# hedgepigdaniel/video-annotator

Hardware: AMD Instinct MI355X
Metric: stabilized frames/sec at 4K NV12, 1/2/4/8 GPU; remap % HBM roofline (higher is better)
Workload: dtype u8 pixels / f32 map / f64 rotations

## Files before the change

### video-annotator_amd/csrc/vstab_testhooks.cpp

```cpp
#include <algorithm>

#include "vstab_hostlogic.hpp"
#include "vstab_pipeline.hpp"
#include "vstab_track_host.hpp"

using namespace vstab;

extern "C" {
__attribute__((visibility("default"))) int vstabx_parse_records(const uint32_t *rec, int n, uint32_t seq, int expect_n, float *xy, unsigned char *status,
                                                                 int *n_out, int *next) {
    std::vector<float> pts;
    std::vector<uint8_t> st;
    int nx = 0;
    const LkParse r = lk_parse_records(rec, 0, n, seq, (size_t)expect_n, pts, st, &nx);
    for (size_t i = 0; i < st.size(); i++) xy[2 * i] = pts[2 * i], xy[2 * i + 1] = pts[2 * i + 1], status[i] = st[i];
    *n_out = (int)st.size(), *next = nx;
    return (int)r;
}
__attribute__((visibility("default"))) int vstabx_dmabuf_cache_sim(const unsigned long long *ids, const size_t *sizes, int n, int cap, long window,
                                                                    long long fail_id, long *counts, unsigned long long *bases) {
    DmaBufCache<unsigned long long> cache;
    cache.cap = cap;
    long destroys = 0, peak = 0;
    std::vector<unsigned long long> live;
    int failures = 0;
    for (int i = 0; i < n; i++) {
        uint8_t *base = nullptr;
        const unsigned long long id = ids[i];
        const bool ok = cache.lookup(id, sizes ? sizes[i] : 4096, window,
                                     [&](unsigned long long &h, uint8_t *&b) {
                                         if ((long long)id == fail_id) return false;
                                         h = id, b = reinterpret_cast<uint8_t *>(static_cast<uintptr_t>(id * 4096));
                                         live.push_back(id);
                                         return true;
                                     },
                                     [&](unsigned long long &h) {
                                         destroys++;
                                         for (size_t k = 0; k < live.size(); k++)
                                             if (live[k] == h) {
                                                 live.erase(live.begin() + (long)k);
                                                 break;
                                             }
                                     },
                                     base);
        failures += !ok;
        bases[i] = ok ? static_cast<unsigned long long>(reinterpret_cast<uintptr_t>(base)) : ~0ull;
        peak = std::max<long>(peak, (long)cache.size());
    }
    counts[0] = cache.imports, counts[1] = cache.evictions, counts[2] = (long)cache.size(), counts[3] = destroys, counts[4] = peak;
    cache.clear([&](unsigned long long &) { destroys++; });
    counts[5] = destroys;
    return failures;
}

__attribute__((visibility("default"))) int vstabx_lk_segments(const void *const *frames, const size_t *pitches, int w, int h, const float *pts, int n,
                                                               const int *seg, int n_seg, const void *const *uv, const size_t *uv_pitches,
                                                               void *const *rings, int bad_parent, uint32_t *host_rec, uint32_t *dev_rec,
                                                               uint8_t *pyr_out, void *stream) {
    if (!frames || !pitches || !pts || !seg || !host_rec || !dev_rec || w <= 0 || h <= 0 || n <= 0 || n_seg <= 0 || n_seg > Tracker::REC_BUFS)
        return fail(VSTAB_ERR_INVALID, "vstabx_lk_segments: bad argument");
    int K = 0;
    for (int s = 0; s < n_seg; s++) {
        if (seg[s] < 1 || seg[s] > LK_SEG_MAX) return fail(VSTAB_ERR_INVALID, "vstabx_lk_segments: a launch covers 1 .. LK_SEG_MAX frame pairs");
        K += seg[s];
    }
    if (K > Tracker::REC_BUFS) return fail(VSTAB_ERR_INVALID, "vstabx_lk_segments: more frame pairs than record buffers");
    if (bad_parent != -1 && (bad_parent < 1 || bad_parent >= n_seg)) return fail(VSTAB_ERR_INVALID, "vstabx_lk_segments: bad_parent is not a chained launch");
    const bool pack = uv || uv_pitches || rings;
    if (pack && (!uv || !uv_pitches || !rings)) return fail(VSTAB_ERR_INVALID, "vstabx_lk_segments: uv, uv_pitches and rings go together");
    if (pack && lk_levels(w, h) < 2) return fail(VSTAB_ERR_INVALID, "vstabx_lk_segments: a one-level pyramid has no level 1 to pack");
    for (int i = 0; i <= K; i++) {
        if (!frames[i] || pitches[i] < (size_t)w || pitches[i] >= (1u << 24) || (uint64_t)pitches[i] * (uint64_t)h >= (1ull << 32))
            return fail(VSTAB_ERR_INVALID, "vstabx_lk_segments: bad frame");
        if (pack && (!uv[i] || !rings[i] || !pack_pyr_ok(frames[i], pitches[i], uv[i], uv_pitches[i], w, h, rings[i], rings[i], (size_t)((w + 1) / 2))))
            return fail(VSTAB_ERR_INVALID, "vstabx_lk_segments: planes not aligned for the fused copy");
    }
    hipStream_t st = static_cast<hipStream_t>(stream);
    Tracker t;
    VSTAB_TRY(t.init(w, h));
    VSTAB_TRY(t.reserve_slots(n));
    const int levels = t.levels();
    size_t pyr_bytes = 0;
    for (int l = 1; l < levels; l++) pyr_bytes += (size_t)t.level_w(l) * t.level_h(l);
    std::vector<LkPyramid> pyr(K + 1);
    int built = -1;
    auto build = [&](int i) -> vstab_status {
        const int s = i % PYR_SETS;
        const uint8_t *y = static_cast<const uint8_t *>(frames[i]);
        size_t pitch = pitches[i];
        if (pack) {
            uint8_t *ring = static_cast<uint8_t *>(rings[i]);
            VSTAB_TRY(launch_pack_pyr(y, pitch, static_cast<const uint8_t *>(uv[i]), uv_pitches[i], w, h, ring, t.level1(s), t.level1_pitch(), st));
            y = ring, pitch = (size_t)w;
        }
        VSTAB_TRY(t.build_pyramid(s, y, pitch, st, nullptr, nullptr, pack));
        pyr[i] = t.pyramid(s, y, pitch);
        if (pyr_out) {
            uint8_t *o = pyr_out + pyr_bytes * i;
            for (int l = 1; l < levels; l++) {
                const size_t lw = (size_t)t.level_w(l), lh = (size_t)t.level_h(l);
                VSTAB_HIP_TRY(hipMemcpyAsync(o, pyr[i].img[l], lw * lh, hipMemcpyDeviceToHost, st));
                o += lw * lh;
            }
        }
        built = i;
        return VSTAB_OK;
    };
    std::vector<Tracker::Launch> launches(n_seg);
    std::vector<float> start(pts, pts + 2 * (size_t)n);
    int first = 0;
    for (int s = 0; s < n_seg; s++) {
        for (int i = built + 1; i <= first + seg[s]; i++) VSTAB_TRY(build(i));
        if (s == 0) {
            VSTAB_TRY(t.track_launch(&pyr[first], seg[s], start, st, false, launches[s]));
        } else {
            Tracker::Launch parent = launches[s - 1];
            if (s == bad_parent) parent.seq[parent.n_frames - 1] ^= 0x40u;
            VSTAB_TRY(t.track_launch_chained(&pyr[first], seg[s], parent, st, launches[s]));
        }
        first += seg[s];
    }
    VSTAB_HIP_TRY(hipStreamSynchronize(st));
    int k = 0;
    for (int s = 0; s < n_seg; s++)
        for (int i = 0; i < seg[s]; i++, k++) {
            std::memcpy(host_rec + (size_t)k * n * 4, t.host_records(launches[s], i), (size_t)n * 16);
            VSTAB_HIP_TRY(hipMemcpy(dev_rec + (size_t)k * n * 4, t.dev_records(launches[s], i), (size_t)n * 16, hipMemcpyDeviceToHost));
        }
    return VSTAB_OK;
}

__attribute__((visibility("default"))) int vstabx_corners_fused(const void *gray, size_t pitch, int w, int h, double quality, unsigned int cap, unsigned int canary,
                                                                 unsigned long long *keys_out, unsigned int *counts_out, unsigned int *tile_counts,
                                                                 void *stream) {
    if (!gray || !keys_out || !counts_out || !tile_counts) return fail(VSTAB_ERR_INVALID, "vstabx_corners_fused: bad argument");
    if (w < 3 || h < 3 || pitch < (size_t)w) return fail(VSTAB_ERR_INVALID, "vstabx_corners_fused: an image is at least 3 x 3 and its pitch at least its width");
    if ((uint64_t)pitch * (uint64_t)h >= (1ull << 32) || (uint64_t)w * (uint64_t)h >= (1ull << 31))
        return fail(VSTAB_ERR_INVALID, "vstabx_corners_fused: planes of 4 GiB or more and images of 2^31 pixels or more are not supported");
    if (!(quality > 0.0) || !(quality <= 1.0)) return fail(VSTAB_ERR_INVALID, "vstabx_corners_fused: quality lies in (0, 1]");
    if (cap < 1 || cap > (1u << 24)) return fail(VSTAB_ERR_INVALID, "vstabx_corners_fused: cap is 1 .. 2^24 keys");
    if (canary < 1 || canary > (1u << 16)) return fail(VSTAB_ERR_INVALID, "vstabx_corners_fused: canary is 1 .. 2^16 keys");
    hipStream_t st = static_cast<hipStream_t>(stream);
    const size_t tiles = (size_t)div_up((unsigned)w, 64u) * div_up((unsigned)h, 31u), scratch_bytes = corners_fused_scratch_bytes(w, h);
    if (scratch_bytes != tiles * (256 * sizeof(unsigned long long) + 64 * 31 * sizeof(float) + sizeof(unsigned int)))
        return fail(VSTAB_ERR_DEVICE, "vstabx_corners_fused: the scratch layout of launch_corners_fused is not the one this hook reads");
    const size_t n_keys = (size_t)cap + canary;
    DevBuf scratch, keys, small;
    VSTAB_TRY(scratch.ensure(scratch_bytes));
    VSTAB_TRY(keys.ensure(n_keys * sizeof(unsigned long long)));
    VSTAB_TRY(small.ensure(256));
    VSTAB_HIP_TRY(hipMemsetAsync(scratch.p, 0, scratch_bytes, st));
    VSTAB_HIP_TRY(hipMemsetAsync(keys.p, 0xA5, n_keys * sizeof(unsigned long long), st));
    VSTAB_TRY(launch_corners_fused(static_cast<const uint8_t *>(gray), pitch, w, h, quality, scratch.p, keys.as<unsigned long long>(), cap, small.as<unsigned int>(), st));
    VSTAB_HIP_TRY(hipMemcpyAsync(keys_out, keys.p, n_keys * sizeof(unsigned long long), hipMemcpyDeviceToHost, st));
    VSTAB_HIP_TRY(hipMemcpyAsync(counts_out, small.as<unsigned int>() + 4, 2 * sizeof(unsigned int), hipMemcpyDeviceToHost, st));
    VSTAB_HIP_TRY(hipMemcpyAsync(tile_counts, scratch.as<uint8_t>() + (scratch_bytes - tiles * sizeof(unsigned int)), tiles * sizeof(unsigned int), hipMemcpyDeviceToHost, st));
    VSTAB_HIP_TRY(hipStreamSynchronize(st));
    return VSTAB_OK;
}

__attribute__((visibility("default"))) int vstabx_detector_counters(const vstab_handle *h, long *out) {
    if (!h || !out) return fail(VSTAB_ERR_INVALID, "vstabx_detector_counters: bad argument");
    out[0] = h->tracker.spec_over_cap(), out[1] = h->tracker.fused_overflows(), out[2] = (long)h->tracker.key_capacity();
    return VSTAB_OK;
}
}
```

### video-annotator_amd/csrc/vstab_warp_fused.hip

```cpp
#include <algorithm>
#include <climits>
#include <cmath>
#include <cstdlib>

#include "vstab_device10.hpp"
#include "vstab_warp_host.hpp"
#include "vstab_warp_tile.hpp"

namespace vstab {

#ifdef VSTAB_DEV
#define VSTAB_STAMP(k)                                                                                                   \
    if (ta.timing && lane == 0) ta.timing[((size_t)blockIdx.x * 4 + (size_t)wave) * 8 + (k)] = __builtin_amdgcn_s_memrealtime()
#else
#define VSTAB_STAMP(k)
#endif

template <int RWB, int RW, int MODE, int FMT, bool CACHED, bool SPLIT, int DEPTH = 8, int BLEND = 0>
__device__ __forceinline__ bool warp_tile(const FusedArgs &ta, uint32_t *smem, const int x0, const int y0) {
    static_assert((DEPTH == 8 && FMT < 2) || (DEPTH == 10 && FMT >= 2), "10-bit pixels leave as 16-bit BGR (FMT 2) or P010 planes (FMT 3)");
    using SrcVec = typename std::conditional<DEPTH == 10, uint4, uint2>::type;
    constexpr uint32_t BPS = DEPTH == 10 ? 2 : 1;
    constexpr int TH = 4 * RW;
    constexpr int STAGE_MAX = StageTrips<RWB, RW>::value;
    constexpr int QB = CACHED ? 0 : QMAGIC_BITS;
    constexpr bool PIX8 = DEPTH == 10 && BLEND == VSTAB_BLEND_FP16;
    constexpr int PD = PIX8 ? 2 : 1;
    constexpr bool RS = map_mode_is_rs(MODE);
    constexpr int BASE = map_mode_base(MODE);
    uint32_t *const tile = smem + 8;
    const WarpArgs &a = ta.w;
    const int tid = threadIdx.x, lane = tid & 63, wave = __builtin_amdgcn_readfirstlane(tid >> 6);
    const float rfx = rcp_refined(a.p.ofx), rfy = rcp_refined(a.p.ofy);

    VSTAB_STAMP(0);
    if (wave == 0) {
        __builtin_amdgcn_s_setprio(3);
        probe_tile<TH, STAGE_MAX, MODE, CACHED>(ta, x0, y0, lane, rfx, rfy, smem);
        __builtin_amdgcn_s_setprio(VSTAB_WARP_PRIO);
    }
    __syncthreads();
    const int bx0 = __builtin_amdgcn_readfirstlane((int)smem[0]), by0 = __builtin_amdgcn_readfirstlane((int)smem[1]);
    const int wb = __builtin_amdgcn_readfirstlane((int)smem[2]), hb = __builtin_amdgcn_readfirstlane((int)smem[3]);
    const int box_state = __builtin_amdgcn_readfirstlane((int)smem[4]);
    if constexpr (SPLIT) {
        if (box_state == 2) return false;
    }
    const bool use_lds = box_state == 1;
    const int x = x0 + lane;
    VSTAB_STAMP(1);

    const int ux_n = wb >> 3, units = use_lds ? ux_n * (hb >> 1) : 0;
#ifdef VSTAB_DEV
    const int pw = (wb + ta.lds_pad) * PD;
#else
    const int pw = wb * PD;
#endif
    SrcVec y0w[STAGE_MAX], y1w[STAGE_MAX], uvw[STAGE_MAX];
    int ldsoff[STAGE_MAX];
    constexpr int ZERO_BLOCK = 1 << 24;
    if (use_lds) {
        const float rn = __builtin_amdgcn_rcpf((float)ux_n);
        int uy = (int)((float)tid * rn), ux = tid - uy * ux_n;
        if (ux < 0) ux += ux_n, uy--;
        if (ux >= ux_n) ux -= ux_n, uy++;
        int sy_ = (int)(256.0f * rn), sx_ = 256 - sy_ * ux_n;
        if (sx_ < 0) sx_ += ux_n, sy_--;
        if (sx_ >= ux_n) sx_ -= ux_n, sy_++;
        const uint32_t pitch_y = (uint32_t)a.pitch_y, pitch_uv = (uint32_t)a.pitch_uv;
#pragma unroll
        for (int it = 0; it < STAGE_MAX; it++) {
            if (it > 0 && units <= it * 256) {
                y0w[it] = y1w[it] = uvw[it] = SrcVec(), ldsoff[it] = -1;
                continue;
            }
            const bool valid = tid + it * 256 < units;
            const int gx = bx0 + 8 * ux, gy = by0 + 2 * uy;
            const bool inside = (uint32_t)gx < (uint32_t)(a.sw & ~7) && (uint32_t)gy < (uint32_t)a.sh;
            const uint32_t cx = (uint32_t)min(max(gx, 0), (a.sw & ~7) - 8), cy = (uint32_t)min(max(gy, 0), a.sh - 2);
            const uint32_t oy = __umul24(cy, pitch_y) + cx * BPS, ouv = __umul24(cy >> 1, pitch_uv) + cx * BPS;
            y0w[it] = *reinterpret_cast<const SrcVec *>(a.y + oy);
            y1w[it] = *reinterpret_cast<const SrcVec *>(a.y + (oy + pitch_y));
            uvw[it] = *reinterpret_cast<const SrcVec *>(a.uv + ouv);
            ldsoff[it] = valid ? (__mul24(2 * uy, pw) + 8 * PD * ux) | (inside ? 0 : ZERO_BLOCK) : -1;
            ux += sx_, uy += sy_;
            if (ux >= ux_n) ux -= ux_n, uy++;
        }
    } else {
#pragma unroll
        for (int it = 0; it < STAGE_MAX; it++) y0w[it] = y1w[it] = uvw[it] = SrcVec(), ldsoff[it] = -1;
    }

    VSTAB_STAMP(2);
    int qxb[RW], qyb[RW];
    {
        int unused_cx[RW / 2], unused_cy[RW / 2];
        const float unused_qm[4] = {QMAGIC, QMAGIC, QMAGIC, QMAGIC};
        map_phase<RW, MODE, CACHED, false>(ta, x, y0, wave, lane, rfx, rfy, qxb, qyb, unused_cx, unused_cy, unused_qm);
    }
#pragma unroll
    for (int j = 0; j < RW; j++) asm volatile("" : "+v"(qxb[j]), "+v"(qyb[j]) : : "memory");

    VSTAB_STAMP(3);
    if (use_lds) {
#pragma unroll
        for (int it = 0; it < STAGE_MAX; it++) {
            if (ldsoff[it] >= ZERO_BLOCK) {
                uint32_t *d = tile + (ldsoff[it] - ZERO_BLOCK);
                const uint4 z = make_uint4(0, 0, 0, 0);
#pragma unroll
                for (int q = 0; q < 2 * PD; q++) *reinterpret_cast<uint4 *>(d + 4 * q) = z, *reinterpret_cast<uint4 *>(d + pw + 4 * q) = z;
#ifdef VSTAB_DEV
            } else if (DEPTH == 8 && ldsoff[it] >= 0 && (ta.ablate & 4)) {
                uint32_t *d = tile + ldsoff[it];
                *reinterpret_cast<uint4 *>(d) = make_uint4(y0w[it].x, y0w[it].y, uvw[it].x, uvw[it].y);
                *reinterpret_cast<uint4 *>(d + 4) = make_uint4(y0w[it].y, y0w[it].x, uvw[it].x, uvw[it].y);
                *reinterpret_cast<uint4 *>(d + pw) = make_uint4(y1w[it].x, y1w[it].y, uvw[it].x, uvw[it].y);
                *reinterpret_cast<uint4 *>(d + pw + 4) = make_uint4(y1w[it].y, y1w[it].x, uvw[it].y, uvw[it].x);
#endif
            } else if (ldsoff[it] >= 0) {
                uint32_t *d = tile + ldsoff[it];
                if constexpr (DEPTH == 10) {
                    const uint32_t ya[4] = {y0w[it].x, y0w[it].y, y0w[it].z, y0w[it].w}, yb[4] = {y1w[it].x, y1w[it].y, y1w[it].z, y1w[it].w};
                    const uint32_t cw[4] = {uvw[it].x, uvw[it].y, uvw[it].z, uvw[it].w};
#pragma unroll
                    for (int half = 0; half < 2; half++) {
                        const ChromaTerm c0 = chroma_term10(cw[2 * half]), c1 = chroma_term10(cw[2 * half + 1]);
                        if constexpr (PIX8) {
                            const uint32_t la = ya[2 * half], lb = ya[2 * half + 1], ma = yb[2 * half], mb = yb[2 * half + 1];
                            const uint2 a0 = pack_bgr10h((int)((la & 0xffffu) >> 6), c0), a1 = pack_bgr10h((int)(la >> 22), c0);
                            const uint2 a2 = pack_bgr10h((int)((lb & 0xffffu) >> 6), c1), a3 = pack_bgr10h((int)(lb >> 22), c1);
                            const uint2 b0 = pack_bgr10h((int)((ma & 0xffffu) >> 6), c0), b1 = pack_bgr10h((int)(ma >> 22), c0);
                            const uint2 b2 = pack_bgr10h((int)((mb & 0xffffu) >> 6), c1), b3 = pack_bgr10h((int)(mb >> 22), c1);
                            *reinterpret_cast<uint4 *>(d + 8 * half) = make_uint4(a0.x, a0.y, a1.x, a1.y);
                            *reinterpret_cast<uint4 *>(d + 8 * half + 4) = make_uint4(a2.x, a2.y, a3.x, a3.y);
                            *reinterpret_cast<uint4 *>(d + pw + 8 * half) = make_uint4(b0.x, b0.y, b1.x, b1.y);
                            *reinterpret_cast<uint4 *>(d + pw + 8 * half + 4) = make_uint4(b2.x, b2.y, b3.x, b3.y);
                            continue;
                        }
                        uint4 r0, r1;
                        r0.x = pack_bgr10((int)((ya[2 * half] & 0xffffu) >> 6), c0), r0.y = pack_bgr10((int)(ya[2 * half] >> 22), c0);
                        r0.z = pack_bgr10((int)((ya[2 * half + 1] & 0xffffu) >> 6), c1), r0.w = pack_bgr10((int)(ya[2 * half + 1] >> 22), c1);
                        r1.x = pack_bgr10((int)((yb[2 * half] & 0xffffu) >> 6), c0), r1.y = pack_bgr10((int)(yb[2 * half] >> 22), c0);
                        r1.z = pack_bgr10((int)((yb[2 * half + 1] & 0xffffu) >> 6), c1), r1.w = pack_bgr10((int)(yb[2 * half + 1] >> 22), c1);
                        *reinterpret_cast<uint4 *>(d + 4 * half) = r0;
                        *reinterpret_cast<uint4 *>(d + pw + 4 * half) = r1;
                    }
                } else
#pragma unroll
                for (int half = 0; half < 2; half++) {
                    const uint32_t cw = half ? uvw[it].y : uvw[it].x, ya = half ? y0w[it].y : y0w[it].x, yb = half ? y1w[it].y : y1w[it].x;
                    const ChromaTerm c0 = chroma_term_folded(cw & 255, (cw >> 8) & 255);
                    const ChromaTerm c1 = chroma_term_folded((cw >> 16) & 255, cw >> 24);
                    uint4 r0, r1;
                    r0.x = pack_bgrx(ya & 255, c0), r0.y = pack_bgrx((ya >> 8) & 255, c0);
                    r0.z = pack_bgrx((ya >> 16) & 255, c1), r0.w = pack_bgrx(ya >> 24, c1);
                    r1.x = pack_bgrx(yb & 255, c0), r1.y = pack_bgrx((yb >> 8) & 255, c0);
                    r1.z = pack_bgrx((yb >> 16) & 255, c1), r1.w = pack_bgrx(yb >> 24, c1);
                    *reinterpret_cast<uint4 *>(d + 4 * half) = r0;
                    *reinterpret_cast<uint4 *>(d + pw + 4 * half) = r1;
                }
            }
        }
    }
    VSTAB_STAMP(4);
    __syncthreads();
    VSTAB_STAMP(5);

    const bool col_live = x < a.dw;
    uint32_t out[RW];
    {
        int cx = bx0 + (QB >> 5), cy = by0 + (QB >> 5);
        asm("" : "+s"(cx), "+s"(cy));
        const uint32_t wlim = use_lds ? (uint32_t)(wb - 1) : 0u, hlim = (uint32_t)(hb - 1);
        int Xr[RW], Yr[RW];
        const uint32_t wb4 = (uint32_t)pw << 2;
        uint32_t tile_lds = (uint32_t)(uintptr_t)(__attribute__((address_space(3))) uint32_t *)tile;
        asm("" : "+s"(tile_lds));
        uint32_t mxx = 0, mxy = 0;
#pragma unroll
        for (int j = 0; j < RW; j++) {
            Xr[j] = (qxb[j] >> 5) - cx, Yr[j] = (qyb[j] >> 5) - cy;
            mxx = max(mxx, (uint32_t)Xr[j]), mxy = max(mxy, (uint32_t)Yr[j]);
        }
        if (!__builtin_amdgcn_ballot_w64(mxx >= wlim || mxy >= hlim)) {
            constexpr int TG = RW < TAP_GROUP ? RW : TAP_GROUP;
            if constexpr (PIX8) {
#pragma unroll
                for (int j0 = 0; j0 < RW; j0 += TG) {
                    uint2 t0[TG], t1[TG], t2[TG], t3[TG];
#pragma unroll
                    for (int j = 0; j < TG; j++) {
                        uint32_t ax8, au;
                        asm("v_lshl_add_u32 %0, %1, 3, %2" : "=v"(ax8) : "v"(Xr[j0 + j]), "s"(tile_lds));
                        asm("v_mad_u32_u24 %0, %1, %2, %3" : "=v"(au) : "v"(Yr[j0 + j]), "s"(wb4), "v"(ax8));
                        const LdsPair *u = reinterpret_cast<const LdsPair *>(au), *l = reinterpret_cast<const LdsPair *>(au + wb4);
                        const u32x2 v0 = u[0], v1 = u[1], v2 = l[0], v3 = l[1];
                        t0[j] = make_uint2(v0.x, v0.y), t1[j] = make_uint2(v1.x, v1.y), t2[j] = make_uint2(v2.x, v2.y), t3[j] = make_uint2(v3.x, v3.y);
                    }
#pragma unroll
                    for (int j = 0; j < TG; j++) out[j0 + j] = blend_bgr10h(t0[j], t1[j], t2[j], t3[j], qxb[j0 + j] & 31, qyb[j0 + j] & 31);
                }
            } else
#pragma unroll
            for (int j0 = 0; j0 < RW; j0 += TG) {
                uint32_t t0[TG], t1[TG], t2[TG], t3[TG];
#pragma unroll
                for (int j = 0; j < TG; j++) {
                    uint32_t ax4, au;
                    asm("v_lshl_add_u32 %0, %1, 2, %2" : "=v"(ax4) : "v"(Xr[j0 + j]), "s"(tile_lds));
                    asm("v_mad_u32_u24 %0, %1, %2, %3" : "=v"(au) : "v"(Yr[j0 + j]), "s"(wb4), "v"(ax4));
                    const LdsWord *u = reinterpret_cast<const LdsWord *>(au), *l = reinterpret_cast<const LdsWord *>(au + wb4);
                    t0[j] = u[0], t1[j] = u[1], t2[j] = l[0], t3[j] = l[1];
                }
#pragma unroll
                for (int j = 0; j < TG; j++) {
#ifdef VSTAB_DEV
                    if (ta.ablate & 2) out[j0 + j] = t0[j] ^ t1[j] ^ t2[j] ^ t3[j] ^ (qxb[j0 + j] & 31) ^ (qyb[j0 + j] & 31);
                    else
#endif
                    out[j0 + j] = DEPTH == 10 ? blend_bgr10<BLEND>(t0[j], t1[j], t2[j], t3[j], qxb[j0 + j] & 31, qyb[j0 + j] & 31)
                                              : blend_bgrx(t0[j], t1[j], t2[j], t3[j], qxb[j0 + j] & 31, qyb[j0 + j] & 31);
                }
            }
        } else {
            uint32_t slow = 0;
#pragma unroll
            for (int j = 0; j < RW; j++) {
                const bool inbox = (uint32_t)Xr[j] < wlim && (uint32_t)Yr[j] < hlim;
                uint32_t v = 0;
                if (inbox) {
                    const uint32_t *t = tile + (__mul24(Yr[j], pw) + PD * Xr[j]);
                    if constexpr (PIX8)
                        v = blend_bgr10h(make_uint2(t[0], t[1]), make_uint2(t[2], t[3]), make_uint2(t[pw], t[pw + 1]), make_uint2(t[pw + 2], t[pw + 3]), qxb[j] & 31,
                                         qyb[j] & 31);
                    else
                        v = DEPTH == 10 ? blend_bgr10<BLEND>(t[0], t[1], t[pw], t[pw + 1], qxb[j] & 31, qyb[j] & 31)
                                        : blend_bgrx(t[0], t[1], t[pw], t[pw + 1], qxb[j] & 31, qyb[j] & 31);
                }
                out[j] = v;
                const bool live = col_live && y0 + wave * RW + j < a.dh;
                slow |= (!inbox && live ? 1u : 0u) << j;
            }
            if (__builtin_amdgcn_ballot_w64(slow != 0)) {
#pragma unroll 1
                for (int j = 0; j < RW; j++) {
                    int sx = qxb[0], sy = qyb[0];
#pragma unroll
                    for (int k = 1; k < RW; k++) sx = j == k ? qxb[k] : sx, sy = j == k ? qyb[k] : sy;
                    if ((slow >> j) & 1u) {
                        const uint32_t v = DEPTH == 10 ? gather_pixel10<BLEND>(a, sx - QB, sy - QB) : gather_pixel_far(a, sx - QB, sy - QB);
#pragma unroll
                        for (int k = 0; k < RW; k++) out[k] = j == k ? v : out[k];
                    }
// ... 134 lines not shown
    return true;
}

template <int RWB, int MODE, int FMT, bool CACHED, int DEPTH = 8, int BLEND = 0>
__global__ void __launch_bounds__(256, DEPTH == 10 ? 5 : (RWB == 8 || map_mode_is_rs(MODE)) ? VSTAB_WARP_WAVES - 1 : VSTAB_WARP_WAVES) k_warp_fused(FusedArgs ta) {
    extern __shared__ __attribute__((aligned(16))) uint32_t smem[];
    constexpr int TH = 4 * RWB, TS = TH / 2;
    if (VSTAB_WARP_PRIO) __builtin_amdgcn_s_setprio(VSTAB_WARP_PRIO);
    const int k = (int)(blockIdx.x & 7u);
    const int y_lo = ta.band_y[k], y_sp = ta.split_y[k], y_hi = ta.band_y[k + 1];
    const int n_tall = ((y_sp - y_lo) / TH) * ta.tiles_x;
    const int idx = (int)(blockIdx.x >> 3);
    int x0, ys, n_half;
    if (idx < n_tall) {
        const int row = idx / ta.tiles_x;
        x0 = (idx - row * ta.tiles_x) * 64, ys = y_lo + row * TH;
        n_half = warp_tile<RWB, RWB, MODE, FMT, CACHED, true, DEPTH, BLEND>(ta, smem, x0, ys) ? 0 : 2;
    } else {
        const int i2 = idx - n_tall, row = i2 / ta.tiles_x;
        x0 = (i2 - row * ta.tiles_x) * 64, ys = y_sp + row * TS, n_half = 1;
        if (ys >= y_hi) return;
    }
#pragma unroll 1
    for (int i = 0; i < n_half; i++) warp_tile<RWB, RWB / 2, MODE, FMT, CACHED, false, DEPTH, BLEND>(ta, smem, x0, ys + i * TS);
}

}

using namespace vstab;

namespace vstab {
#ifdef VSTAB_DEV
static unsigned long long *g_dev_timing = nullptr;
extern "C" __attribute__((visibility("default"))) void vstab_dev_set_timing(void *p) { g_dev_timing = static_cast<unsigned long long *>(p); }
#endif

vstab_status launch_warp_fused10(const WarpArgs &a, const float params[17], int map_mode, int blend, const float *rot_bottom, bool p010_out, bool src_vec_ok,
                                 bool dst_vec_ok, hipStream_t st) {
    FusedArgs ta;
    fill_fused_args(ta, a, params, src_vec_ok, dst_vec_ok, nullptr, 0, rot_bottom);
    const int lds_kb = 40;
    const bool half = blend == VSTAB_BLEND_FP16;
    const int rwb = 8;
    const long tiles = (long)div_up(a.dw, 64) * div_up(a.dh, 4 * rwb);
    const dim3 grid(tile_schedule(ta, rwb, lds_kb, tiles > 1024 ? 0.5 : 0.0));
    if (half) ta.lds_capacity_px /= 2;
    const size_t lds_bytes = (size_t)lds_kb * 1024;
    vstab_status status = VSTAB_OK;
    with_map_mode(map_mode, rot_bottom != nullptr, [&](auto mode) {
        with_either<VSTAB_BLEND_FP16, VSTAB_BLEND_EXACT>(half, [&](auto blend_c) {
            with_either<3, 2>(p010_out, [&](auto fmt) {
                constexpr int MODE = decltype(mode)::value;
                if constexpr (map_mode_fish_to_pinhole(map_mode_base(MODE)))
                    launch_kernel(k_warp_fused<8, MODE, decltype(fmt)::value, false, 10, decltype(blend_c)::value>, grid, dim3(256), lds_bytes, st, ta);
                else
                    status = fail(VSTAB_ERR_INVALID, "launch_warp_fused10: the 10-bit tiled kernels serve map modes 0, 1 and 5 only");
            });
        });
    });
    if (status != VSTAB_OK) return status;
    VSTAB_HIP_TRY(hipGetLastError());
    return VSTAB_OK;
}

vstab_status launch_warp_fused(const WarpArgs &a, const float params[17], int map_mode, bool nv12_out, bool src_vec_ok, bool dst_vec_ok,
                               const void *qmap, int qpitch, const float *rot_bottom, hipStream_t st, const float *dist) {
    FusedArgs ta;
    fill_fused_args(ta, a, params, src_vec_ok, dst_vec_ok, qmap, qpitch, rot_bottom, dist);
#ifdef VSTAB_DEV
    ta.timing = g_dev_timing;
    static const int ablate = getenv("VSTAB_ABLATE") ? atoi(getenv("VSTAB_ABLATE")) : 0;
    ta.ablate = ablate;
    ta.lds_pad = getenv("VSTAB_LDS_PAD") ? atoi(getenv("VSTAB_LDS_PAD")) & ~3 : 0;
#endif
    const long tiles32 = (long)div_up(a.dw, 64) * div_up(a.dh, 32);
    int rwb = tiles32 < 1536 ? 4 : 8, lds_kb = rwb == 4 ? 20 : 40;
    double tail_rounds = (double)div_up(a.dw, 64) * div_up(a.dh, 4 * rwb) > 256.0 * (160 / lds_kb) ? 0.5 : 0.0;
#ifdef VSTAB_DEV
    if (const char *e = getenv("VSTAB_ROWS")) rwb = atoi(e) == 4 ? 4 : 8;
    if (const char *e = getenv("VSTAB_LDS_KB")) lds_kb = atoi(e);
    if (const char *e = getenv("VSTAB_TAIL_ROUNDS")) tail_rounds = atof(e);
#endif
    const size_t lds_bytes = (size_t)lds_kb * 1024;
    const dim3 grid(tile_schedule(ta, rwb, lds_kb, tail_rounds));
    if (dist) {
        if (nv12_out || qmap || rot_bottom) return fail(VSTAB_ERR_INVALID, "launch_warp_fused: the distorted-lens kernels emit BGR8 from one rotation per frame");
        with_dist_mode(map_mode, [&](auto mode) {
            with_either<8, 4>(rwb == 8, [&](auto rows) {
                launch_kernel(k_warp_fused<decltype(rows)::value, decltype(mode)::value, 0, false>, grid, dim3(256), lds_bytes, st, ta);
            });
        });
        VSTAB_HIP_TRY(hipGetLastError());
        return VSTAB_OK;
    }
    with_map_mode(qmap ? (int)VSTAB_MAP_CREATEMAP_CL : map_mode, !qmap && rot_bottom != nullptr, [&](auto mode) {
        with_bool(qmap != nullptr, [&](auto cached) {
            with_either<8, 4>(rwb == 8, [&](auto rows) {
                with_either<1, 0>(nv12_out, [&](auto fmt) {
                    constexpr int MODE = decltype(mode)::value;
                    constexpr bool CACHED = decltype(cached)::value;
                    if constexpr (!CACHED || MODE == MAP_CREATEMAP_CL)
                        launch_kernel(k_warp_fused<decltype(rows)::value, MODE, decltype(fmt)::value, CACHED>, grid, dim3(256), lds_bytes, st, ta);
                });
            });
        });
    });
    VSTAB_HIP_TRY(hipGetLastError());
    return VSTAB_OK;
}


vstab_status preload_fused_kernels() {
    hipFuncAttributes at;
    VSTAB_HIP_TRY(hipFuncGetAttributes(&at, reinterpret_cast<const void *>((&k_warp_fused<8, MAP_CREATEMAP_CL_OPENCL, 0, false, 8, 0>))));
    return VSTAB_OK;
}

}
```

### video-annotator_amd/csrc/vstab_warp_tile.hpp

```cpp
#pragma once
#include <algorithm>
#include <climits>
#include <cmath>
#include <cstdlib>

#include "vstab_device.hpp"
#include "vstab_internal.hpp"
#include "vstab_warp_args.hpp"

namespace vstab {

#ifndef VSTAB_WARP_WAVES
#define VSTAB_WARP_WAVES 7
#endif
#ifndef VSTAB_WARP_PRIO
#define VSTAB_WARP_PRIO 1
#endif
#ifndef VSTAB_MAP_GROUP
#define VSTAB_MAP_GROUP 2
#endif
#ifndef VSTAB_TAP_GROUP
#define VSTAB_TAP_GROUP 4
#endif
constexpr int MAP_GROUP = VSTAB_MAP_GROUP;
constexpr int TAP_GROUP = VSTAB_TAP_GROUP;
constexpr float QMAGIC = 12582912.0f;
constexpr int QMAGIC_BITS = 0x4B400000;

typedef short short2v __attribute__((ext_vector_type(2)));
typedef __attribute__((address_space(3))) uint32_t LdsWord;
typedef uint32_t u32x2 __attribute__((ext_vector_type(2)));
typedef __attribute__((address_space(3))) u32x2 LdsPair;

__device__ __forceinline__ uint32_t pk_min_i16(uint32_t a, uint32_t b) {
    return __builtin_bit_cast(uint32_t, __builtin_elementwise_min(__builtin_bit_cast(short2v, a), __builtin_bit_cast(short2v, b)));
}
__device__ __forceinline__ uint32_t pk_max_i16(uint32_t a, uint32_t b) {
    return __builtin_bit_cast(uint32_t, __builtin_elementwise_max(__builtin_bit_cast(short2v, a), __builtin_bit_cast(short2v, b)));
}

template <bool MAX>
__device__ __forceinline__ uint32_t wave_reduce_pk_i16(uint32_t v) {
    constexpr uint32_t ident = MAX ? 0x80008000u : 0x7fff7fffu;
#define VSTAB_STEP(ctrl, rmask)                                                                              \
    {                                                                                                        \
        const uint32_t t = (uint32_t)__builtin_amdgcn_update_dpp((int)ident, (int)v, ctrl, rmask, 0xf, false); \
        v = MAX ? pk_max_i16(v, t) : pk_min_i16(v, t);                                                       \
    }
    VSTAB_STEP(0x111, 0xf) VSTAB_STEP(0x112, 0xf) VSTAB_STEP(0x114, 0xf) VSTAB_STEP(0x118, 0xf)
    VSTAB_STEP(0x142, 0xa) VSTAB_STEP(0x143, 0xc)
#undef VSTAB_STEP
    return (uint32_t)__builtin_amdgcn_readlane((int)v, 63);
}

__device__ __forceinline__ uint32_t gather_pixel_far(const WarpArgs &a, int sx, int sy) {
    const int X = sx >> 5, Y = sy >> 5;
    if (!(X < a.sw && X + 1 >= 0 && Y < a.sh && Y + 1 >= 0)) return 0;
    return gather_pixel(a, sx, sy);
}

template <int RWB, int RW>
struct StageTrips {
    static constexpr int value = RW == 8 ? 3 : RW == 4 ? 2 : (RWB == 8 ? 2 : 1);
};

template <int TH, int STAGE_MAX, int MODE, bool CACHED, bool PLANAR = false, int BLOCK_W = 8>
__device__ __forceinline__ void probe_tile(const FusedArgs &ta, int x0, int y0, int lane, float rfx, float rfy, uint32_t *hdr) {
    constexpr bool RS = map_mode_is_rs(MODE);
    constexpr int BASE = map_mode_base(MODE);
    const WarpArgs &a = ta.w;
    int px, py;
    const int l16 = lane & 15, side = (l16 * (TH - 1) + 7) / 15;
    if (lane < 16) px = 4 * l16, py = 0;
    else if (lane < 32) px = 4 * l16 + 3, py = TH - 1;
    else if (lane < 48) px = 0, py = side;
    else px = 63, py = side;
    px = min(px, a.dw - 1 - x0), py = min(py, a.dh - 1 - y0);
    int qx, qy;
    if constexpr (CACHED) {
        const int2 q = ta.qmap[(size_t)(y0 + py) * ta.qpitch + (x0 + px)];
        qx = q.x, qy = q.y;
    } else {
        float ax, ay;
        if constexpr (BASE == MAP_CREATEMAP_CL || BASE == MAP_FISH_TO_RECT || BASE == MAP_CREATEMAP_CL_OPENCL || BASE == MAP_FISHD_TO_RECT) {
            const float vx = ((float)(x0 + px) - a.p.ocx) * rfx, vy = ((float)(y0 + py) - a.p.ocy) * rfy;
            float m[9];
#pragma unroll
            for (int k = 0; k < 9; k++) m[k] = a.p.r[k];
            if constexpr (RS) {
                const float t = (float)(y0 + py) * __builtin_amdgcn_rcpf(ta.rs_den);
#pragma unroll
                for (int k = 0; k < 9; k++) m[k] = __builtin_fmaf(t, ta.rs_d[k], a.p.r[k]);
            }
            const float wx = __builtin_fmaf(m[0], vx, __builtin_fmaf(m[1], vy, m[2]));
            const float wy = __builtin_fmaf(m[3], vx, __builtin_fmaf(m[4], vy, m[5]));
            const float wz = __builtin_fmaf(m[6], vx, __builtin_fmaf(m[7], vy, m[8]));
            const float rz = __builtin_amdgcn_rcpf(wz), ux = wx * rz, uy = wy * rz;
            const float q = __builtin_fmaf(ux, ux, uy * uy), rs = __builtin_amdgcn_rsqf(q), rad = q * rs;
            const bool inv = rad > 1.0f;
            const float t = inv ? rs : rad, s2 = t * t;
            float g = 0.0028423243202269077f;
            g = __builtin_fmaf(g, s2, -0.016053270548582077f);
            g = __builtin_fmaf(g, s2, 0.04269874095916748f);
            g = __builtin_fmaf(g, s2, -0.07508683204650879f);
            g = __builtin_fmaf(g, s2, 0.1064559817314148f);
            g = __builtin_fmaf(g, s2, -0.14205896854400635f);
            g = __builtin_fmaf(g, s2, 0.19993145763874054f);
            g = __builtin_fmaf(g, s2, -0.33333125710487366f);
            float at = __builtin_fmaf(t * s2, g, t);
            at = inv ? 1.57079637050628662109375f - at : at;
            if constexpr (BASE == MAP_FISHD_TO_RECT) {
                const Distortion &dk = ta.p32.d;
                const float a2 = at * at;
                const float pd = __builtin_fmaf(__builtin_fmaf(__builtin_fmaf(dk.k4, a2, dk.k3), a2, dk.k2), a2, dk.k1);
                at = at * __builtin_fmaf(pd, a2, 1.0f);
            }
            const float k = at * rs;
            ax = __builtin_fmaf(ux * k, ta.p32.ifx32, ta.p32.icx32), ay = __builtin_fmaf(uy * k, ta.p32.ify32, ta.p32.icy32);
            if ((BASE == MAP_FISH_TO_RECT || BASE == MAP_FISHD_TO_RECT) && !(wz > 0.0f)) ax = ay = __builtin_nanf("");
        } else {
            const float vx = div_with_rcp((float)(x0 + px) - a.p.ocx, a.p.ofx, rfx);
            const float vy = div_with_rcp((float)(y0 + py) - a.p.ocy, a.p.ofy, rfy);
            const ColTerm ct = {a.p.r[0] * vx, a.p.r[3] * vx, a.p.r[6] * vx};
            const RowTerm rt = {a.p.r[1] * vy, a.p.r[4] * vy, a.p.r[7] * vy};
            map_pixel_ex<BASE>(ta.p32, a.p, ct, rt, vx, vy, ax, ay);
        }
        qx = __float_as_int(ax + QMAGIC) - QMAGIC_BITS, qy = __float_as_int(ay + QMAGIC) - QMAGIC_BITS;
    }
    int Xc, Yc;
    asm("v_med3_i32 %0, %1, -1, %2" : "=v"(Xc) : "v"(qx >> 5), "s"(a.sw));
    asm("v_med3_i32 %0, %1, -1, %2" : "=v"(Yc) : "v"(qy >> 5), "s"(a.sh));
    const uint32_t pk = ((uint32_t)Xc & 0xffffu) | ((uint32_t)Yc << 16);
    const uint32_t mn = wave_reduce_pk_i16<false>(pk), mx = wave_reduce_pk_i16<true>(pk);
    const int mnx = (int)(short)(mn & 0xffffu), mny = (int)mn >> 16, mxx = (int)(short)(mx & 0xffffu), mxy = (int)mx >> 16;
    constexpr int LO_M = PLANAR ? 2 : 1, HI_M = PLANAR ? 5 : 2, CAP = PLANAR ? 1 : 0, BM = BLOCK_W - 1;
    const int lox = max(mnx - LO_M, -LO_M), hix = min(mxx + HI_M, a.sw + CAP), loy = max(mny - LO_M, -LO_M), hiy = min(mxy + HI_M, a.sh + CAP);
    const int bx0 = lox & ~BM, by0 = loy & ~1;
    const int wb = (hix + 1 - bx0 + BM) & ~BM, hb = (hiy + 1 - by0 + 1) & ~1;
    const bool have = mnx < a.sw && mxx >= -1 && mny < a.sh && mxy >= -1;
    const bool stageable = have && a.sw >= BLOCK_W && ta.src_vec_ok && ((a.sw & BM) == 0 || bx0 + wb <= (a.sw & ~BM));
#ifdef VSTAB_DEV
    const bool fits = (wb + ta.lds_pad) * hb <= ta.lds_capacity_px && (wb >> 3) * (hb >> 1) <= STAGE_MAX * 256;
#else
    const bool fits = wb * hb <= ta.lds_capacity_px && (wb / BLOCK_W) * (hb >> 1) <= STAGE_MAX * 256 && (!PLANAR || wb / BLOCK_W <= 64);
#endif
    if (lane == 0) {
        *reinterpret_cast<uint4 *>(hdr) = make_uint4((uint32_t)bx0, (uint32_t)by0, (uint32_t)wb, (uint32_t)hb);
        hdr[4] = stageable ? (fits ? 1u : 2u) : 0u;
    }
}

#define VSTAB_EACH _Pragma("unroll") for (int c = 0; c < NP; c++)
template <int NP, bool FISH_TO_RECT, bool DIST = false>
__device__ __forceinline__ void map_pairs_ieee(float icx32, float icy32, float ifx32, float ify32, const f32x2 (&wx)[NP], const f32x2 (&wy)[NP],
                                               const f32x2 (&wz)[NP], f32x2 (&ax)[NP], f32x2 (&ay)[NP], const Distortion &dk = Distortion()) {
    f32x2 rz[NP], e[NP], px[NP], py[NP], ex[NP], ey[NP], q[NP], y[NP], g[NP], h[NP], d[NP], rad[NP], rr[NP], t[NP], s[NP], at[NP], k[NP];
    i32x2 inv[NP];
    const f32x2 one = splat2(1.0f), half = splat2(0.5f);
    VSTAB_EACH rz[c] = (f32x2){__builtin_amdgcn_rcpf(wz[c].x), __builtin_amdgcn_rcpf(wz[c].y)};
    VSTAB_EACH e[c] = fma2(-wz[c], rz[c], one);
    VSTAB_EACH rz[c] = fma2(e[c], rz[c], rz[c]);
    VSTAB_EACH px[c] = wx[c] * rz[c], py[c] = wy[c] * rz[c];
    VSTAB_EACH ex[c] = fma2(-wz[c], px[c], wx[c]), ey[c] = fma2(-wz[c], py[c], wy[c]);
    VSTAB_EACH px[c] = fma2(ex[c], rz[c], px[c]), py[c] = fma2(ey[c], rz[c], py[c]);
    VSTAB_EACH ex[c] = fma2(-wz[c], px[c], wx[c]), ey[c] = fma2(-wz[c], py[c], wy[c]);
    VSTAB_EACH px[c] = fma2(ex[c], rz[c], px[c]), py[c] = fma2(ey[c], rz[c], py[c]);
    VSTAB_EACH q[c] = px[c] * px[c] + py[c] * py[c];
    VSTAB_EACH y[c] = (f32x2){__builtin_amdgcn_rsqf(q[c].x), __builtin_amdgcn_rsqf(q[c].y)};
    VSTAB_EACH g[c] = q[c] * y[c], h[c] = half * y[c];
    VSTAB_EACH e[c] = fma2(-h[c], g[c], half);
    VSTAB_EACH h[c] = fma2(h[c], e[c], h[c]), g[c] = fma2(g[c], e[c], g[c]);
    VSTAB_EACH d[c] = fma2(-g[c], g[c], q[c]);
    VSTAB_EACH rad[c] = fma2(d[c], h[c], g[c]);
    VSTAB_EACH rr[c] = (f32x2){__builtin_amdgcn_rcpf(rad[c].x), __builtin_amdgcn_rcpf(rad[c].y)};
    VSTAB_EACH e[c] = fma2(-rad[c], rr[c], one);
    VSTAB_EACH rr[c] = fma2(e[c], rr[c], rr[c]);
    VSTAB_EACH inv[c] = rad[c] > one, t[c] = one * rr[c];
    VSTAB_EACH e[c] = fma2(-rad[c], t[c], one);
    VSTAB_EACH t[c] = fma2(e[c], rr[c], t[c]);
    VSTAB_EACH e[c] = fma2(-rad[c], t[c], one);
    VSTAB_EACH t[c] = fma2(e[c], rr[c], t[c]);
    VSTAB_EACH t[c] = inv[c] ? t[c] : rad[c];
    VSTAB_EACH s[c] = t[c] * t[c];
    VSTAB_EACH g[c] = fma2(splat2(0.0028423243202269077f), s[c], splat2(-0.016053270548582077f));
    VSTAB_EACH g[c] = fma2(g[c], s[c], splat2(0.04269874095916748f));
    VSTAB_EACH g[c] = fma2(g[c], s[c], splat2(-0.07508683204650879f));
    VSTAB_EACH g[c] = fma2(g[c], s[c], splat2(0.1064559817314148f));
    VSTAB_EACH g[c] = fma2(g[c], s[c], splat2(-0.14205896854400635f));
    VSTAB_EACH g[c] = fma2(g[c], s[c], splat2(0.19993145763874054f));
    VSTAB_EACH g[c] = fma2(g[c], s[c], splat2(-0.33333125710487366f));
    VSTAB_EACH at[c] = fma2(t[c] * s[c], g[c], t[c]);
    VSTAB_EACH at[c] = inv[c] ? (splat2(1.57079637050628662109375f) - at[c]) + splat2(-4.37113900018624283e-8f) : at[c];
    if constexpr (DIST) {
        VSTAB_EACH s[c] = at[c] * at[c];
        VSTAB_EACH g[c] = splat2(dk.k4) * s[c];
        VSTAB_EACH g[c] = g[c] + splat2(dk.k3);
        VSTAB_EACH g[c] = g[c] * s[c];
        VSTAB_EACH g[c] = g[c] + splat2(dk.k2);
        VSTAB_EACH g[c] = g[c] * s[c];
        VSTAB_EACH g[c] = g[c] + splat2(dk.k1);
        VSTAB_EACH g[c] = g[c] * s[c];
        VSTAB_EACH g[c] = one + g[c];
        VSTAB_EACH at[c] = at[c] * g[c];
    }
    VSTAB_EACH k[c] = at[c] * rr[c];
    VSTAB_EACH e[c] = fma2(-rad[c], k[c], at[c]);
    VSTAB_EACH k[c] = fma2(e[c], rr[c], k[c]);
    VSTAB_EACH e[c] = fma2(-rad[c], k[c], at[c]);
    VSTAB_EACH k[c] = fma2(e[c], rr[c], k[c]);
    if constexpr (FISH_TO_RECT) {
        VSTAB_EACH k[c] = (q[c] == splat2(0.0f)) ? one : k[c];
    }
    VSTAB_EACH ax[c] = splat2(icx32) + (px[c] * k[c]) * splat2(ifx32), ay[c] = splat2(icy32) + (py[c] * k[c]) * splat2(ify32);
    if constexpr (FISH_TO_RECT) {
        VSTAB_EACH {
            const i32x2 ok = wz[c] > splat2(0.0f);
            ax[c] = ok ? ax[c] : splat2(__builtin_nanf("")), ay[c] = ok ? ay[c] : splat2(__builtin_nanf(""));
        }
    }
}

__device__ __forceinline__ bool map_q_irregular(uint32_t qmin, uint32_t qmax) { return qmin < 0x17800000u  || qmax > 0x67800000u ; }
template <int NP>
__device__ __forceinline__ void map_pairs_ocl(float icx32, float icy32, float ifx32, float ify32, const f32x2 (&wx)[NP], const f32x2 (&wy)[NP],
                                              const f32x2 (&wz)[NP], f32x2 (&ax)[NP], f32x2 (&ay)[NP], uint32_t &qmin, uint32_t &qmax) {
    f32x2 rz[NP], px[NP], py[NP], q[NP], rad[NP], rr[NP], t[NP], s[NP], p[NP], r[NP], k[NP];
    i32x2 inv[NP];
    VSTAB_EACH rz[c] = (f32x2){__builtin_amdgcn_rcpf(wz[c].x), __builtin_amdgcn_rcpf(wz[c].y)};
    VSTAB_EACH px[c] = wx[c] * rz[c], py[c] = wy[c] * rz[c];
    VSTAB_EACH q[c] = fma2(py[c], py[c], px[c] * px[c]);
    VSTAB_EACH rad[c] = (f32x2){__builtin_amdgcn_sqrtf(q[c].x), __builtin_amdgcn_sqrtf(q[c].y)};
// ... 189 lines not shown
```

Measured before the change: 28220.

## Add cost-weighted band scheduling and dead-tile skip for fisheye warp

Adds a host-side cost model that estimates, per tile row, how much source footprint the projection touches. It uses that estimate to place the eight band boundaries so each band gets balanced work instead of equal rows, and caches the schedule for rotations within a small angle. On the device, the probe wave now checks whether a whole tile maps well outside the source image. If so, the tile skips map and sample work and writes zeros. This trades a host-side geometric estimate and a conservative device-side guard for less imbalance and less wasted gather work, but risks wrong zero tiles if the margin heuristics are too loose.

Measured after the change: 30480 (median of 6 runs). +8.0%, better.

```diff
diff --git a/video-annotator_amd/csrc/vstab_testhooks.cpp b/video-annotator_amd/csrc/vstab_testhooks.cpp
--- a/video-annotator_amd/csrc/vstab_testhooks.cpp
+++ b/video-annotator_amd/csrc/vstab_testhooks.cpp
@@ -3,6 +3,7 @@
 #include "vstab_hostlogic.hpp"
 #include "vstab_pipeline.hpp"
 #include "vstab_track_host.hpp"
+#include "vstab_warp_bands.hpp"
 
 using namespace vstab;
 
@@ -159,6 +160,44 @@
     return VSTAB_OK;
 }
 
+__attribute__((visibility("default"))) int vstabx_weighted_bands(int dw, int dh, int rwb, int lds_kb, double tail_rounds, const uint32_t *cost, int n_cost,
+                                                                  int *out) {
+    if (!out || dw < 1 || dh < 1 || (rwb != 4 && rwb != 8) || lds_kb < 1 || !(tail_rounds >= 0.0) || n_cost < 0)
+        return fail(VSTAB_ERR_INVALID, "vstabx_weighted_bands: bad argument");
+    FusedArgs ta = {};
+    ta.w.dw = dw, ta.w.dh = dh;
+    const unsigned grid = cost ? weighted_bands(ta, rwb, lds_kb, tail_rounds, cost, n_cost) : tile_schedule(ta, rwb, lds_kb, tail_rounds);
+    for (int k = 0; k < 9; k++) out[k] = ta.band_y[k];
+    for (int k = 0; k < 8; k++) out[9 + k] = ta.split_y[k];
+    out[17] = ta.tiles_x, out[18] = (int)grid;
+    return VSTAB_OK;
+}
+__attribute__((visibility("default"))) int vstabx_band_costs(const float *params, int nan_behind, int sw, int sh, int dw, int dh, int ts, uint32_t *cost, int n_cost) {
+    if (!params || !cost || sw < 1 || sh < 1 || dw < 1 || dh < 1 || (ts != 8 && ts != 16) || n_cost != (int)div_up((unsigned)dh, (unsigned)ts))
+        return fail(VSTAB_ERR_INVALID, "vstabx_band_costs: bad argument");
+    std::vector<uint32_t> c;
+    band_costs(params, nan_behind != 0, sw, sh, dw, dh, ts, c);
+    std::copy(c.begin(), c.end(), cost);
+    return VSTAB_OK;
+}
+__attribute__((visibility("default"))) int vstabx_band_cache_run(const float *params, int n, int sw, int sh, int dw, int dh, int map_mode, int rwb, int lds_kb,
+                                                                  double tail_rounds, int *out, long *counts) {
+    if (!params || !out || !counts || n < 1 || sw < 1 || sh < 1 || dw < 1 || dh < 1 || (rwb != 4 && rwb != 8) || lds_kb < 1 || !(tail_rounds >= 0.0))
+        return fail(VSTAB_ERR_INVALID, "vstabx_band_cache_run: bad argument");
+    BandCache cache;
+    for (int i = 0; i < n; i++) {
+        FusedArgs ta = {};
+        ta.w.sw = sw, ta.w.sh = sh, ta.w.dw = dw, ta.w.dh = dh;
+        const unsigned grid = cache.schedule(ta, params + 17 * (size_t)i, map_mode, rwb, lds_kb, tail_rounds);
+        int *o = out + 19 * (size_t)i;
+        for (int k = 0; k < 9; k++) o[k] = ta.band_y[k];
+        for (int k = 0; k < 8; k++) o[9 + k] = ta.split_y[k];
+        o[17] = ta.tiles_x, o[18] = (int)grid;
+    }
+    counts[0] = cache.hits, counts[1] = cache.misses, counts[2] = (long)cache.entries.size();
+    return VSTAB_OK;
+}
+
 __attribute__((visibility("default"))) int vstabx_detector_counters(const vstab_handle *h, long *out) {
     if (!h || !out) return fail(VSTAB_ERR_INVALID, "vstabx_detector_counters: bad argument");
     out[0] = h->tracker.spec_over_cap(), out[1] = h->tracker.fused_overflows(), out[2] = (long)h->tracker.key_capacity();
diff --git a/video-annotator_amd/csrc/vstab_warp_bands.hpp b/video-annotator_amd/csrc/vstab_warp_bands.hpp
--- /dev/null
+++ b/video-annotator_amd/csrc/vstab_warp_bands.hpp
@@ -0,0 +1,139 @@
+#pragma once
+#include <array>
+#include <cmath>
+#include <cstdint>
+#include <cstring>
+#include <mutex>
+#include <vector>
+
+#include "vstab_warp_tile.hpp"
+
+namespace vstab {
+
+static inline unsigned weighted_bands(FusedArgs &ta, int rwb, int lds_kb, double tail_rounds, const uint32_t *cost, int n_cost) {
+    const unsigned even_grid = tile_schedule(ta, rwb, lds_kb, tail_rounds);
+    const WarpArgs &a = ta.w;
+    const int th = 4 * rwb, ts = th / 2;
+    const int half_rows = (int)div_up(a.dh, ts);
+    if (!cost || n_cost != half_rows) return even_grid;
+    uint64_t total = 0;
+    for (int i = 0; i < half_rows; i++) total += cost[i];
+    if (total == 0) return even_grid;
+    const int slots = 32 * std::max(1, std::min(8, (int)(160 / lds_kb)));
+    int h = 0;
+    uint64_t prefix = 0;
+    ta.band_y[0] = 0;
+    for (int k = 1; k < 8; k++) {
+        while (h < half_rows && 8 * (prefix + cost[h]) <= (uint64_t)k * total) prefix += cost[h++];
+        ta.band_y[k] = std::min(a.dh, h * ts);
+    }
+    ta.band_y[8] = a.dh;
+    int share = 0;
+    for (int k = 0; k < 8; k++) {
+        const int rows = ta.band_y[k + 1] - ta.band_y[k];
+        const int tall_rows_max = rows / th;
+        const int tail_tall_rows = (int)std::min<long>(tall_rows_max, std::lround(tail_rounds * slots / ta.tiles_x));
+        const int tall_rows = tall_rows_max - tail_tall_rows;
+        ta.split_y[k] = ta.band_y[k] + tall_rows * th;
+        const int n = tall_rows * ta.tiles_x + (int)div_up(ta.band_y[k + 1] - ta.split_y[k], ts) * ta.tiles_x;
+        share = std::max(share, n);
+    }
+    return 8u * (unsigned)share;
+}
+
+constexpr uint32_t BAND_COST_DEAD = 135, BAND_COST_LIVE = 220;
+constexpr double BAND_COST_PER_BLOCK = 0.58;
+
+static inline void band_costs(const float params[17], bool nan_behind, int sw, int sh, int dw, int dh, int ts, std::vector<uint32_t> &cost) {
+    const int tiles_x = (int)div_up(dw, 64), half_rows = (int)div_up(dh, ts);
+    const double icx = params[0], icy = params[1], ifx = params[2], ify = params[3], ocx = params[4], ocy = params[5], ofx = params[6], ofy = params[7];
+    const float *r = params + 8;
+    std::vector<double> X((size_t)(tiles_x + 1) * 2), Y((size_t)(tiles_x + 1) * 2);
+    auto corners = [&](int row, double *xo, double *yo) {
+        const double vy = ((double)std::min(row * ts, dh - 1) - ocy) / ofy;
+        for (int c = 0; c <= tiles_x; c++) {
+            const double vx = ((double)std::min(c * 64, dw - 1) - ocx) / ofx;
+            const double wx = r[0] * vx + r[1] * vy + r[2], wy = r[3] * vx + r[4] * vy + r[5], wz = r[6] * vx + r[7] * vy + r[8];
+            if (!(wz > 0.0) && (nan_behind || wz == 0.0)) {
+                xo[c] = yo[c] = NAN;
+                continue;
+            }
+            const double ux = wx / wz, uy = wy / wz, rad = std::sqrt(ux * ux + uy * uy), k = rad > 0.0 ? std::atan(rad) / rad : 1.0;
+            xo[c] = icx + ifx * ux * k, yo[c] = icy + ify * uy * k;
+        }
+    };
+    cost.assign((size_t)half_rows, 0u);
+    double *x0 = X.data(), *x1 = x0 + tiles_x + 1, *y0 = Y.data(), *y1 = y0 + tiles_x + 1;
+    corners(0, x0, y0);
+    for (int row = 0; row < half_rows; row++) {
+        corners(row + 1, x1, y1);
+        uint32_t sum = 0;
+        for (int c = 0; c < tiles_x; c++) {
+            const double xs[4] = {x0[c], x0[c + 1], x1[c], x1[c + 1]}, ys[4] = {y0[c], y0[c + 1], y1[c], y1[c + 1]};
+            double mnx = xs[0], mxx = xs[0], mny = ys[0], mxy = ys[0];
+            bool finite = true;
+            for (int i = 0; i < 4; i++) {
+                finite = finite && std::isfinite(xs[i]) && std::isfinite(ys[i]);
+                mnx = std::min(mnx, xs[i]), mxx = std::max(mxx, xs[i]), mny = std::min(mny, ys[i]), mxy = std::max(mxy, ys[i]);
+            }
+            double blocks = 64.0 * ts * 4.0 / 16.0;
+            if (finite) {
+                if (mxx < -1.0 || mnx >= (double)sw || mxy < -1.0 || mny >= (double)sh) {
+                    sum += BAND_COST_DEAD;
+                    continue;
+                }
+                const double bw = std::min(mxx + 2.0, (double)sw) - std::max(mnx - 1.0, -1.0) + 8.0;
+                const double bh = std::min(mxy + 2.0, (double)sh) - std::max(mny - 1.0, -1.0) + 2.0;
+                blocks = std::max(bw, 8.0) * std::max(bh, 2.0) / 16.0;
+            }
+            sum += BAND_COST_LIVE + (uint32_t)std::min(blocks * BAND_COST_PER_BLOCK, 4096.0);
+        }
+        cost[(size_t)row] = sum;
+        std::swap(x0, x1), std::swap(y0, y1);
+    }
+}
+
+constexpr double BAND_CACHE_ANGLE = 1.5 * 3.14159265358979323846 / 180.0;
+constexpr int BAND_CACHE_ENTRIES = 32;
+struct BandCache {
+    struct Entry {
+        float fixed[8];
+        int dims[8];
+        float rot[9];
+        int band_y[9], split_y[8];
+        unsigned grid;
+    };
+    std::mutex mu;
+    std::vector<Entry> entries;
+    size_t next = 0;
+    long hits = 0, misses = 0;
+
+    unsigned schedule(FusedArgs &ta, const float params[17], int map_mode, int rwb, int lds_kb, double tail_rounds) {
+        const WarpArgs &a = ta.w;
+        const int dims[8] = {a.sw, a.sh, a.dw, a.dh, map_mode, rwb, lds_kb, (int)std::lround(tail_rounds * 64.0)};
+        const double min_trace = 1.0 + 2.0 * std::cos(BAND_CACHE_ANGLE);
+        std::lock_guard<std::mutex> lock(mu);
+        for (const Entry &e : entries) {
+            if (std::memcmp(e.fixed, params, sizeof e.fixed) || std::memcmp(e.dims, dims, sizeof dims)) continue;
+            double tr = 0.0;
+            for (int i = 0; i < 9; i++) tr += (double)e.rot[i] * params[8 + i];
+            if (!(tr >= min_trace)) continue;
+            tile_schedule(ta, rwb, lds_kb, tail_rounds);
+            std::memcpy(ta.band_y, e.band_y, sizeof e.band_y), std::memcpy(ta.split_y, e.split_y, sizeof e.split_y);
+            hits++;
+            return e.grid;
+        }
+        misses++;
+        std::vector<uint32_t> cost;
+        band_costs(params, map_mode == MAP_FISH_TO_RECT, a.sw, a.sh, a.dw, a.dh, 2 * rwb, cost);
+        Entry e;
+        std::memcpy(e.fixed, params, sizeof e.fixed), std::memcpy(e.dims, dims, sizeof dims), std::memcpy(e.rot, params + 8, sizeof e.rot);
+        e.grid = weighted_bands(ta, rwb, lds_kb, tail_rounds, cost.data(), (int)cost.size());
+        std::memcpy(e.band_y, ta.band_y, sizeof e.band_y), std::memcpy(e.split_y, ta.split_y, sizeof e.split_y);
+        if ((int)entries.size() < BAND_CACHE_ENTRIES) entries.push_back(e);
+        else entries[next++ % BAND_CACHE_ENTRIES] = e;
+        return e.grid;
+    }
+};
+
+}
diff --git a/video-annotator_amd/csrc/vstab_warp_fused.hip b/video-annotator_amd/csrc/vstab_warp_fused.hip
--- a/video-annotator_amd/csrc/vstab_warp_fused.hip
+++ b/video-annotator_amd/csrc/vstab_warp_fused.hip
@@ -4,6 +4,7 @@
 #include <cstdlib>
 
 #include "vstab_device10.hpp"
+#include "vstab_warp_bands.hpp"
 #include "vstab_warp_host.hpp"
 #include "vstab_warp_tile.hpp"
 
@@ -28,6 +29,7 @@
     constexpr int PD = PIX8 ? 2 : 1;
     constexpr bool RS = map_mode_is_rs(MODE);
     constexpr int BASE = map_mode_base(MODE);
+    constexpr bool DEAD = !CACHED && !RS && (BASE == MAP_CREATEMAP_CL || BASE == MAP_CREATEMAP_CL_OPENCL || BASE == MAP_FISH_TO_RECT);
     uint32_t *const tile = smem + 8;
     const WarpArgs &a = ta.w;
     const int tid = threadIdx.x, lane = tid & 63, wave = __builtin_amdgcn_readfirstlane(tid >> 6);
@@ -36,7 +38,7 @@
     VSTAB_STAMP(0);
     if (wave == 0) {
         __builtin_amdgcn_s_setprio(3);
-        probe_tile<TH, STAGE_MAX, MODE, CACHED>(ta, x0, y0, lane, rfx, rfy, smem);
+        probe_tile<TH, STAGE_MAX, MODE, CACHED, false, 8, DEAD>(ta, x0, y0, lane, rfx, rfy, smem);
         __builtin_amdgcn_s_setprio(VSTAB_WARP_PRIO);
     }
     __syncthreads();
@@ -47,6 +49,7 @@
         if (box_state == 2) return false;
     }
     const bool use_lds = box_state == 1;
+    const bool dead = DEAD && box_state == 3;
     const int x = x0 + lane;
     VSTAB_STAMP(1);
 
@@ -93,7 +96,10 @@
 
     VSTAB_STAMP(2);
     int qxb[RW], qyb[RW];
-    {
+    if (dead) {
+#pragma unroll
+        for (int j = 0; j < RW; j++) qxb[j] = qyb[j] = 0;
+    } else {
         int unused_cx[RW / 2], unused_cy[RW / 2];
         const float unused_qm[4] = {QMAGIC, QMAGIC, QMAGIC, QMAGIC};
         map_phase<RW, MODE, CACHED, false>(ta, x, y0, wave, lane, rfx, rfy, qxb, qyb, unused_cx, unused_cy, unused_qm);
@@ -169,7 +175,10 @@
 
     const bool col_live = x < a.dw;
     uint32_t out[RW];
-    {
+    if (dead) {
+#pragma unroll
+        for (int j = 0; j < RW; j++) out[j] = 0;
+    } else {
         int cx = bx0 + (QB >> 5), cy = by0 + (QB >> 5);
         asm("" : "+s"(cx), "+s"(cy));
         const uint32_t wlim = use_lds ? (uint32_t)(wb - 1) : 0u, hlim = (uint32_t)(hb - 1);
@@ -470,7 +479,13 @@
     if (const char *e = getenv("VSTAB_TAIL_ROUNDS")) tail_rounds = atof(e);
 #endif
     const size_t lds_bytes = (size_t)lds_kb * 1024;
-    const dim3 grid(tile_schedule(ta, rwb, lds_kb, tail_rounds));
+    bool weighted = tail_rounds > 0.0 && !dist && !qmap && !rot_bottom &&
+                    (map_mode == MAP_CREATEMAP_CL || map_mode == MAP_FISH_TO_RECT || map_mode == MAP_CREATEMAP_CL_OPENCL);
+#ifdef VSTAB_DEV
+    if (const char *e = getenv("VSTAB_BANDS")) weighted = weighted && atoi(e) != 0;
+#endif
+    static BandCache band_cache;
+    const dim3 grid(weighted ? band_cache.schedule(ta, params, map_mode, rwb, lds_kb, tail_rounds) : tile_schedule(ta, rwb, lds_kb, tail_rounds));
     if (dist) {
         if (nv12_out || qmap || rot_bottom) return fail(VSTAB_ERR_INVALID, "launch_warp_fused: the distorted-lens kernels emit BGR8 from one rotation per frame");
         with_dist_mode(map_mode, [&](auto mode) {
diff --git a/video-annotator_amd/csrc/vstab_warp_tile.hpp b/video-annotator_amd/csrc/vstab_warp_tile.hpp
--- a/video-annotator_amd/csrc/vstab_warp_tile.hpp
+++ b/video-annotator_amd/csrc/vstab_warp_tile.hpp
@@ -64,7 +64,23 @@
     static constexpr int value = RW == 8 ? 3 : RW == 4 ? 2 : (RWB == 8 ? 2 : 1);
 };
 
-template <int TH, int STAGE_MAX, int MODE, bool CACHED, bool PLANAR = false, int BLOCK_W = 8>
+constexpr int DEAD_MARGIN = 16;
+constexpr int DEAD_GUARD = 3 * DEAD_MARGIN / 4;
+constexpr float DEAD_STRETCH = 1.67f;
+__device__ __forceinline__ bool tile_dead_rule(float ax, float ay, float wz, float rz, float slope32, int sw, int sh) {
+    const float pax = __int_as_float(__builtin_amdgcn_update_dpp(__float_as_int(ax), __float_as_int(ax), 0x111, 0xf, 0xf, false));
+    const float pay = __int_as_float(__builtin_amdgcn_update_dpp(__float_as_int(ay), __float_as_int(ay), 0x111, 0xf, 0xf, false));
+    const bool ok = wz > 0.0f && __builtin_fabsf(ax) < 2097152.0f && __builtin_fabsf(ay) < 2097152.0f &&
+                    __builtin_fabsf(ax - pax) < 32.0f * DEAD_GUARD && __builtin_fabsf(ay - pay) < 32.0f * DEAD_GUARD &&
+                    2.0f * DEAD_STRETCH * slope32 * rz <= 32.0f * (DEAD_MARGIN - 1);
+    const float lo = -32.0f * (1 + DEAD_MARGIN), hx = 32.0f * (float)(sw + DEAD_MARGIN), hy = 32.0f * (float)(sh + DEAD_MARGIN);
+    const uint64_t all = __builtin_amdgcn_ballot_w64(true);
+    const bool side = __builtin_amdgcn_ballot_w64(ax < lo) == all || __builtin_amdgcn_ballot_w64(ax >= hx) == all ||
+                      __builtin_amdgcn_ballot_w64(ay < lo) == all || __builtin_amdgcn_ballot_w64(ay >= hy) == all;
+    return __builtin_amdgcn_ballot_w64(ok) == all && side;
+}
+
+template <int TH, int STAGE_MAX, int MODE, bool CACHED, bool PLANAR = false, int BLOCK_W = 8, bool DEAD = false>
 __device__ __forceinline__ void probe_tile(const FusedArgs &ta, int x0, int y0, int lane, float rfx, float rfy, uint32_t *hdr) {
     constexpr bool RS = map_mode_is_rs(MODE);
     constexpr int BASE = map_mode_base(MODE);
@@ -77,6 +93,7 @@
     else px = 63, py = side;
     px = min(px, a.dw - 1 - x0), py = min(py, a.dh - 1 - y0);
     int qx, qy;
+    bool dead = false;
     if constexpr (CACHED) {
         const int2 q = ta.qmap[(size_t)(y0 + py) * ta.qpitch + (x0 + px)];
         qx = q.x, qy = q.y;
@@ -118,6 +135,7 @@
             const float k = at * rs;
             ax = __builtin_fmaf(ux * k, ta.p32.ifx32, ta.p32.icx32), ay = __builtin_fmaf(uy * k, ta.p32.ify32, ta.p32.icy32);
             if ((BASE == MAP_FISH_TO_RECT || BASE == MAP_FISHD_TO_RECT) && !(wz > 0.0f)) ax = ay = __builtin_nanf("");
+            if constexpr (DEAD) dead = tile_dead_rule(ax, ay, wz, rz, __builtin_fmaxf(ta.p32.ifx32, ta.p32.ify32) * __builtin_fmaxf(rfx, rfy), a.sw, a.sh);
         } else {
             const float vx = div_with_rcp((float)(x0 + px) - a.p.ocx, a.p.ofx, rfx);
             const float vy = div_with_rcp((float)(y0 + py) - a.p.ocy, a.p.ofy, rfy);
@@ -147,6 +165,9 @@
     if (lane == 0) {
         *reinterpret_cast<uint4 *>(hdr) = make_uint4((uint32_t)bx0, (uint32_t)by0, (uint32_t)wb, (uint32_t)hb);
         hdr[4] = stageable ? (fits ? 1u : 2u) : 0u;
+        if constexpr (DEAD) {
+            if (dead) hdr[4] = 3u;
+        }
     }
 }
 
```
